# JeremyCCHsu/vae-npvc

Measured on AMD Instinct MI355X. Metric: SP frames/sec (train step: fwd+bwd+Adam), higher is better.
Workload: dtype f32 tensors and accumulation / bf16x2 operands (16 mantissa bits) on the matrix cores

## Files before the change

vae-npvc_amd/csrc/gfx950_layers.hip:

```cpp
#include <cstdlib>
#include <cstring>
#include <type_traits>

#include "gfx950_convgemm.h"
#include "gfx950_convwgrad.h"
#include "gfx950_dense.h"
#include "gfx950_elem.h"
#include "gfx950_tngemm.h"
#include "gfx950_toeplitz.h"
#include "gfx950_toep_bf16.h"
#include "gfx950_planegemm.h"
#include "gfx950_ntring.h"
#include "gfx950_viewconv.h"
#include "gfx950_fconv.h"
#include "gfx950_fwgrad.h"
#include "gfx950_fconv_r.h"
#include "gfx950_fbwd.h"
#include "gfx950_lnb_planes.h"
#include "kernels.h"

namespace vaenpvc {
namespace tuned {

#ifndef E1F_T
// ... 1016 lines not shown
    }
  } else generic::bwd_dec_layer(m, P, F, w, G, s, 2);

  const bool gd0_planes = !lnq && F >= 1024 && bwd_on(VAENPVC_SEL_DEC0) && bwd_on(VAENPVC_SEL_DEC1) && cw_bwd(CW_D0, F);
  const bool gd0_only_planes = gd0_planes && fcr_bwd(CV_D0G, F) && rt().planes <= 2;
  auto lnb_dec0 = [&](const float* dy0) {
    const ConvL& pl = m.dec[0];
    if (gd0_only_planes)
      for_planes([&](auto npl) {
        constexpr int NPL = decltype(npl)::value;
        VAENPVC_TIMED("lnb_dec0", s, (launch_ln_bwd_planes<LnbCfg<32, 57>, NPL, CL_GD0, false>(dy0, w.dec_a[0], w.dec_st[0], P + pl.gamma_off, P + pl.beta_off,
                                         w.d_dec_a[0], us(w.cl[CL_GD0]), cl_plane(CL_GD0, F), G + pl.gamma_off, G + pl.beta_off, G + pl.b_off,
                                         w.scratch + Pk::lnpart, F, LWGS, s)));
      });
    else if (gd0_planes)
      for_planes([&](auto npl) {
        constexpr int NPL = decltype(npl)::value;
        VAENPVC_TIMED("lnb_dec0", s, (launch_ln_bwd_planes<LnbCfg<32, 57>, NPL, CL_GD0, true>(dy0, w.dec_a[0], w.dec_st[0], P + pl.gamma_off, P + pl.beta_off,
                                         w.d_dec_a[0], us(w.cl[CL_GD0]), cl_plane(CL_GD0, F), G + pl.gamma_off, G + pl.beta_off, G + pl.b_off,
                                         w.scratch + Pk::lnpart, F, LWGS, s)));
      });
    else
      VAENPVC_TIMED("lnb_dec0", s, launch_ln_bwd<LnbCfg<32, 57>>(dy0, w.dec_a[0], w.dec_st[0], P + pl.gamma_off, P + pl.beta_off, w.d_dec_a[0],
                                       G + pl.gamma_off, G + pl.beta_off, G + pl.b_off, w.scratch + Pk::lnpart, F, LWGS, s, lnq));
  };
  if (bwd_on(VAENPVC_SEL_DEC1) && bwd_on(VAENPVC_SEL_DEC2) && fb_bwd(FB_D1, F)) {
    const ConvL& pl = m.dec[0];
    float* dy0 = dy_cur == w.dy_tmp ? w.d_dec_a[1] : w.dy_tmp;
    if (gd0_only_planes && !abf) {
      const int nwg = (int)fbwd_grid_d1(rt().planes, F);
      fused_bwd(FB_D1, 1, dy_cur, dy0, "dec1_bwd", us(w.cl[CL_GD0]), cl_plane(CL_GD0, F), w.scratch + Pk::lnpart);
      VAENPVC_TIMED("lnb_dec0", s, hipLaunchKernelGGL(k_ln_bwd_reduce, dim3(3 * 32), dim3(256), 0, s, w.scratch + Pk::lnpart, nwg, 32,
                                                       G + pl.gamma_off, G + pl.beta_off, G + pl.b_off));
    } else {
      fused_bwd(FB_D1, 1, dy_cur, dy0, "dec1_bwd");
      lnb_dec0(dy0);
    }
    dec_bias_done[0] = true;
  } else if (bwd_on(VAENPVC_SEL_DEC1)) {
    const ConvL &l = m.dec[1], &pl = m.dec[0];
    WgArgs a{w.d_dec_a[1], nullptr, nullptr, nullptr, w.dec_a[0], w.dec_st[0], P + pl.gamma_off, P + pl.beta_off,
             G + l.w_off, F, 0};
    const bool fg = fc_bwd(CV_D1G, F), vg = !fg && cv_bwd(CV_D1G, F), fw = fw_bwd(CW_D1, F), vw = !fw && cw_bwd(CW_D1, F);
    if (vg || vw) gsplit(CL_GD1, w.d_dec_a[1], "dec1_gsplit");
    if (vw && !fwd_planes(VAENPVC_SEL_DEC1, CV_D1F, F)) asplit(CL_YD0, w.dec_a[0], w.dec_st[0], &pl, "dec1_asplit");
    ready();
    if (fw) fwg(CW_D1, w.dec_a[0], w.dec_st[0], &pl, w.d_dec_a[1], nullptr, nullptr, G + l.w_off, "dec1_wgrad");
    else if (vw) vwgrad(CW_D1, G + l.w_off, "dec1_wgrad");
    else VAENPVC_TIMED("dec1_wgrad", s2, launch_convwgrad<WD1>(a, WGS, s2));
    if (!dec_bias_done[1]) generic::bias_grad(w.d_dec_a[1], G + l.b_off, F, l.cout, l.hout, s);
    if (fg) fdgrad(CV_D1G, w.d_dec_a[1], w.dy_tmp, "dec1_dgrad");
    else if (vg) vdgrad(CV_D1G, w.dy_tmp, "dec1_dgrad");
    else
    VAENPVC_TIMED("dec1_dgrad", s, launch_convgemm<GD1>(conv_args(w.d_dec_a[1], nullptr, nullptr, nullptr, P + l.w_off, nullptr,
                                                                  w.dy_tmp, F), nsplit_for<GD1>(F), s));
    lnb_dec0(w.dy_tmp);
    dec_bias_done[0] = true;
  } else generic::bwd_dec_layer(m, P, F, w, G, s, 1);

  const bool dh_planes = rt().d0g_planes && gd0_only_planes && fcr_otl(CV_D0G, rt().planes) && pg_step(VAENPVC_SEL_MERGE, F) && F >= 64;
  if (bwd_on(VAENPVC_SEL_DEC0)) {
    const ConvL& l = m.dec[0];
    WgArgs a{w.d_dec_a[0], nullptr, nullptr, nullptr, w.h, nullptr, nullptr, nullptr, G + l.w_off, F, 0};
    const bool rg = fcr_bwd(CV_D0G, F), vg = !rg && cv_bwd(CV_D0G, F), vw = cw_bwd(CW_D0, F);
    if ((vg || vw) && !gd0_planes) gsplit(CL_GD0, w.d_dec_a[0], "dec0_gsplit");
    if (vw && !fwd_planes(VAENPVC_SEL_DEC0, CV_D0F, F) && !d0f_leaves_planes(F)) asplit(CL_H, w.h, nullptr, nullptr, "dec0_asplit");
    ready();
    if (vw) vwgrad(CW_D0, G + l.w_off, "dec0_wgrad");
    else VAENPVC_TIMED("dec0_wgrad", s2, launch_convwgrad<WD0>(a, WGS, s2));
    if (!dec_bias_done[0]) generic::bias_grad(w.d_dec_a[0], G + l.b_off, F, l.cout, l.hout, s);
    if (rg) rdgrad(CV_D0G, w.scratch + Pk::cvw + cv_woff(CV_D0G), w.d_dec_a[0], w.d_h, "dec0_dgrad", gd0_only_planes ? w.cl[CL_GD0] : nullptr,
                   dh_planes ? w.pl_dh : nullptr, 1600);
    else if (vg) vdgrad(CV_D0G, w.d_h, "dec0_dgrad");
    else
    VAENPVC_TIMED("dec0_dgrad", s, (F < SMALL_BATCH_FRAMES ? launch_convgemm<GD0s>(conv_args(w.d_dec_a[0], nullptr, nullptr, nullptr, w.scratch + Pk::gd0,
                                                                  nullptr, w.d_h, F), nsplit_for<GD0s>(F), s) : launch_convgemm<GD0>(conv_args(w.d_dec_a[0], nullptr, nullptr, nullptr, w.scratch + Pk::gd0,
                                                                  nullptr, w.d_h, F), nsplit_for<GD0>(F), s)));
  } else generic::bwd_dec_layer(m, P, F, w, G, s, 0);
  if (lnq) flush_ln_reduce(*lnq, s);
  bucket(m.dec[0].w_off, m.n_params);

  if (bwd_on(VAENPVC_SEL_MERGE)) {
    const bool pgm = pg_step(VAENPVC_SEL_MERGE, F);
    if (pgm) {
      for_planes([&](auto npl) {
        constexpr int NPL = decltype(npl)::value;
        if (F >= 64) {
        int nch = 0;
        if (dh_planes) VAENPVC_TIMED("merge_dsplit", s, (nch = launch_segsum_planes<NPL, MERGE_NY>(us(w.pl_dh), (int64_t)F * 1600, y, 1539, 1600, F, w.dy_tmp, s)));
        else
        VAENPVC_TIMED("merge_dsplit", s, (nch = launch_split_segsum<NPL, MERGE_NY>(w.d_h, y, 1539, 1600, F, us(w.pl_dh), w.dy_tmp, s)));
        VAENPVC_TIMED("merge_segsum", s, launch_sum_parts(w.dy_tmp, nch, MERGE_NY * 1539, w.scratch + Pk::merge_s, s));
        } else {
        SplitArgs sa = split_args(w.d_h, 1539, 1600, F, us(w.pl_dh));
        VAENPVC_TIMED("merge_dsplit", s, launch_split<NPL>(sa, s));
        }
        ready();
        TnpArgs t = tnp_args(w.pl_z, 128, w.pl_dh, 1600, 128, 1539, F, G + m.wz_off, 1539);
        t.tn4 = bwd_on(VAENPVC_SEL_TN_W4);
        VAENPVC_TIMED("merge_wgrad", s2, (launch_gemm_tn<NPL, TN_EPI_PLAIN>(t, TN_WGS_DENSE, s2)));
      });
    } else {
    TnArgs a = tn_args(w.z, 128, w.d_h, 1539, 128, 1539, F, G + m.wz_off, 1539);
    ready();
    VAENPVC_TIMED("merge_wgrad", s2, launch_tngemm(a, false, kchunks_for(F, 13), s2));
    }
    float* Sg = w.scratch + Pk::merge_s;
    if (!(pgm && F >= 64)) {
      (void)hipMemsetAsync(Sg, 0, (size_t)MERGE_NY * 1539 * 4, s);
      int ch = cmax(1, cmin_(cdiv(F, 64), 128)), fc = cdiv(F, ch);
      VAENPVC_TIMED("merge_segsum", s, hipLaunchKernelGGL(k_segsum_atomic<MERGE_NY>, dim3((unsigned)cdiv(1539, 256), (unsigned)cdiv(F, fc)), dim3(256), 0, s,
                                                          w.d_h, y, 1539, F, fc, Sg));
    }
    const int nb_w = cdiv(128 * 1539, 256), nb_e = cdiv(MERGE_NY * 128, 4), nb_b = cdiv(1539, 256);
    VAENPVC_TIMED("merge_small", s, hipLaunchKernelGGL(k_merge_small<MERGE_NY>, dim3((unsigned)(nb_w + nb_e + nb_b)), dim3(256), 0, s, Sg, P + m.emb_off, P + m.wy_off, 128,
                       1539, G + m.wy_off, G + m.emb_off, G + m.bz_off, G + m.by_off, G + m.bm_off, nb_w, nb_e));
    if (pgm) {
      for_planes([&](auto npl) {
        constexpr int NPL = decltype(npl)::value;
        NtArgs a = nt_args(w.pl_dh, F, 1600, w.scratch + Pk::pg_mergeb, 128, 128, w.d_z, 128);
        VAENPVC_TIMED("merge_dgrad", s, launch_gemm_nt<NPL>(a, s));
      });
    } else {
      DenseArgs d = dense_args(w.d_h, w.scratch + Pk::merge_b, w.d_z, 128, F);
      if (F < SMALL_BATCH_FRAMES) {
        (void)hipMemsetAsync(w.d_z, 0, (size_t)F * 128 * 4, s);
        VAENPVC_TIMED("merge_dgrad", s, launch_densegemm<MergeBs>(d, s, 7));
      } else
      VAENPVC_TIMED("merge_dgrad", s, launch_densegemm<MergeB>(d, s));
    }
  } else generic::bwd_merge(m, P, y, F, w, G, s);
  bucket(m.wz_off, m.dec[0].w_off);

  const bool heads_tuned = bwd_on(VAENPVC_SEL_HEADS);
  const bool dz_planes = F >= 1024 && pg_step(VAENPVC_SEL_HEADS, F);
  if (heads_tuned) {
    const int rch = cmax(1, cmin_(cdiv(F, 32), 1024)), rfc = cdiv(F, rch);
    if (dz_planes)
      for_planes([&](auto npl) {
        VAENPVC_TIMED("reparam_bwd", s, hipLaunchKernelGGL((k_reparam_bwd_planes<decltype(npl)::value>), dim3((unsigned)cdiv(F, rfc)), dim3(256), 0, s, w.d_z, w.z_mu,
                           w.z_lv, eps, us(w.pl_dz), w.scratch + Pk::lnpart, (int)F, rfc, 1.0f / (float)F);
                      hipLaunchKernelGGL(k_colsum_part2, dim3(256), dim3(256), 0, s, w.scratch + Pk::lnpart, cdiv(F, rfc), G + m.bmu_off, G + m.blv_off));
      });
    else
    VAENPVC_TIMED("reparam_bwd", s, hipLaunchKernelGGL(k_reparam_bwd_colsum, dim3((unsigned)cdiv(F, rfc)), dim3(256), 0, s, w.d_z, w.z_mu, w.z_lv, eps, w.d_z_mu,
                       w.d_z_lv, G + m.bmu_off, G + m.blv_off, (int)F, rfc, 1.0f / (float)F));
  } else generic::bwd_reparam(m, eps, F, w, s);

  const bool da4_planes = !lnq && F >= 1024 && pg_step(VAENPVC_SEL_HEADS, F) && bwd_on(VAENPVC_SEL_ENC4) && fwd_on(VAENPVC_SEL_ENC4);
  const bool ge3_planes = !lnq && F >= 1024 && bwd_on(VAENPVC_SEL_ENC3) && bwd_on(VAENPVC_SEL_ENC4) && cv_bwd(CV_E3G, F) && cw_bwd(CW_E3, F);
  if (pg_step(VAENPVC_SEL_HEADS, F)) {
    const ConvL& l4 = m.enc[4];
    for_planes([&](auto npl) {
      constexpr int NPL = decltype(npl)::value;
      SplitArgs sa = split_args(w.d_z_mu, 256, 256, F, us(w.pl_dz));
      sa.k1 = 128;
      sa.ld1 = 128;
      sa.src2 = w.d_z_lv;
      sa.ld2 = 128;
      if (!dz_planes) VAENPVC_TIMED("heads_dsplit", s, launch_split<NPL>(sa, s));
      ready();
      TnpArgs t = tnp_args(w.pl_y4, 768, w.pl_dz, 256, 768, 256, F, G + m.wmu_off, 128);
      t.C2 = G + m.wlv_off;
      t.split = 128;
      t.tn4 = bwd_on(VAENPVC_SEL_TN_W4);
      VAENPVC_TIMED("heads_wgrad", s2, (launch_gemm_tn<NPL, TN_EPI_PLAIN>(t, TN_WGS_DENSE, s2)));
      NtArgs a = nt_args(w.pl_dz, F, 256, w.scratch + Pk::pg_headsb, 768, 768, w.dy_tmp, 768);
      VAENPVC_TIMED("heads_dgrad", s, launch_gemm_nt<NPL>(a, s));
    });
    if (da4_planes)
      for_planes([&](auto npl) {
        constexpr int NPL = decltype(npl)::value;
        VAENPVC_TIMED("lnb_enc4", s, (launch_ln_bwd_planes<LnbCfg<256, 3>, NPL, -1, false>(w.dy_tmp, w.enc_a[4], w.enc_st[4], P + l4.gamma_off, P + l4.beta_off,
                                         w.d_enc_a[4], us(w.pl_da4), (int64_t)F * 768, G + l4.gamma_off, G + l4.beta_off, G + l4.b_off,
                                         w.scratch + Pk::lnpart, F, LWGS, s)));
      });
    else
    VAENPVC_TIMED("lnb_enc4", s, launch_ln_bwd<LnbCfg<256, 3>>(w.dy_tmp, w.enc_a[4], w.enc_st[4], P + l4.gamma_off, P + l4.beta_off, w.d_enc_a[4],
                                     G + l4.gamma_off, G + l4.beta_off, G + l4.b_off, w.scratch + Pk::lnpart, F, LWGS, s, lnq));
    enc_bias_done[4] = true;
  } else if (bwd_on(VAENPVC_SEL_HEADS)) {
    const ConvL& l4 = m.enc[4];
    TnArgs a = tn_args(w.enc_a[4], 768, w.d_z_mu, 128, 768, 128, F, G + m.wmu_off, 128);
    a.st = w.enc_st[4];
    a.gamma = P + l4.gamma_off;
    a.beta = P + l4.beta_off;
    a.lndiv = 3;
    ready();
    VAENPVC_TIMED("heads_wgrad", s2, launch_tngemm(a, false, kchunks_for(F, 6), s2));
    a.Y = w.d_z_lv;
    a.C = G + m.wlv_off;
    launch_tngemm(a, false, kchunks_for(F, 6), s2);
    DenseArgs d = dense_args(w.d_z_mu, w.scratch + Pk::heads_b, w.dy_tmp, 768, F);
    d.in2 = w.d_z_lv;
    if (F < SMALL_BATCH_FRAMES) {
      (void)hipMemsetAsync(w.dy_tmp, 0, (size_t)F * 768 * 4, s);
      VAENPVC_TIMED("heads_dgrad", s, launch_densegemm<HeadsBs>(d, s, 4));
    } else
// ... 265 lines not shown
```

vae-npvc_amd/csrc/gfx950_planegemm.h:

```cpp
#pragma once
#include "gfx950_common.h"
#include "gfx950_toep_bf16.h"
#include "philox.h"

namespace vaenpvc {
namespace tuned {

constexpr int PG_KA = 64;

struct RowView {
  int R, fs, x0, step;
};
__device__ __forceinline__ int64_t view_off(const RowView& v, int r) {
  const int f = r / v.R, q = r - f * v.R;
  return (int64_t)f * v.fs + v.x0 + q * v.step;
}
static inline RowView plain_rows(int ld) { return RowView{0x7fffffff, 0, 0, ld}; }

struct SplitArgs {
  const float* src;
  const float* src2;
  int k1, ld1, ld2;
  const float* st;
  const float* gamma;
// ... 846 lines not shown
#pragma unroll
      for (int i = 0; i < 2; ++i)
#pragma unroll
        for (int j = 0; j < 2; ++j) acc[i][j] = mfma_bf16(fa[set][i][PR::A[t]], fb[set][j][PR::B[t]], acc[i][j]);
  };
  constexpr int NKS = NTA_KP / 16;
  auto tile_body = [&](int t, auto full_) __attribute__((always_inline)) {
    constexpr bool FULL = decltype(full_)::value;
    const int n0 = t * NT_BN;
#pragma unroll
    for (int p = 0; p < NPL; ++p)
#pragma unroll
      for (int q = 0; q < NQ; ++q) *reinterpret_cast<u32x4*>(sB + p * BPL + srow * NTA_RS + shalf * NTA_KP + q * 16) = rbq[p][q];
    if constexpr (rb) {
#pragma unroll
      for (int u = 0; u < NTB; ++u) Ts[tid + 256 * u] = tb[u];
    }
    const f32x4 bv = bv4;
    __syncthreads();
    gload(min(t + 1, ntn - 1));
    __builtin_amdgcn_sched_barrier(0);
#pragma unroll
    for (int i = 0; i < 2; ++i)
#pragma unroll
      for (int j = 0; j < 2; ++j) acc[i][j] = zero16();
    loadF(0, 0);
#pragma unroll
    for (int ks = 0; ks < NKS; ++ks) {
      if (ks + 1 < NKS) loadF((ks + 1) & 1, ks + 1);
      __builtin_amdgcn_sched_barrier(0);
      mm(ks & 1);
      __builtin_amdgcn_sched_barrier(0);
    }
    __syncthreads();
    float* ot = reinterpret_cast<float*>(sB);
#pragma unroll
    for (int j = 0; j < 2; ++j)
#pragma unroll
      for (int i = 0; i < 2; ++i)
#pragma unroll
        for (int reg = 0; reg < 16; ++reg)
          ot[(wm * 64 + i * 32 + acc_row(reg, lane)) * NT_EP_PITCH + wn * 64 + j * 32 + l31] = acc[i][j][reg];
    __syncthreads();
    const int pc = tid & 31, r0 = tid >> 5, n = n0 + pc * 4;
    float* cb = a.C + (int64_t)m0 * a.ldc + n;
#pragma unroll
    for (int i = 0; i < NT_BM / 8; ++i) {
      const int row = r0 + 8 * i;
      f32x4 v = *reinterpret_cast<const f32x4*>(ot + row * NT_EP_PITCH + pc * 4);
      v += bv;
      if constexpr (rb) v += *reinterpret_cast<const f32x4*>(Ts + ys[row] * 128 + pc * 4);
      float* o = cb + (int64_t)row * a.ldc;
      if (FULL || n + 3 < a.N) {
        *reinterpret_cast<f32x4_a4*>(o) = f32x4_a4{v[0], v[1], v[2], v[3]};
      } else {
#pragma unroll
        for (int k = 0; k < 4; ++k)
          if (n + k < a.N) o[k] = v[k];
      }
    }
    __syncthreads();
  };
  const int nfull = a.N / NT_BN;
  gload(0);
  tile_body(0, std::true_type{});
  for (int t = 1; t < nfull; ++t) tile_body(t, std::true_type{});
  if (nfull < ntn) tile_body(nfull, std::false_type{});
}
inline bool gemm_nt_ar_serves(const NtArgs& a) {
  return a.Kp == NTA_KP && a.M % NT_BM == 0 && !a.C2 && (!a.rowbias || (a.nrb <= NT_MAXRB && a.idx)) && a.N >= NT_BN;
}
template <int NPL>
inline void launch_gemm_nt_ar(const NtArgs& a, hipStream_t s) {
  if (a.rowbias) {
    rt().ensure_lds(reinterpret_cast<const void*>(&k_gemm_nt_ar<NPL, true>), nta_lds(NPL));
    hipLaunchKernelGGL((k_gemm_nt_ar<NPL, true>), dim3((unsigned)(a.M / NT_BM)), dim3(256), nta_lds(NPL), s, a);
  } else {
    rt().ensure_lds(reinterpret_cast<const void*>(&k_gemm_nt_ar<NPL, false>), nta_lds(NPL));
    hipLaunchKernelGGL((k_gemm_nt_ar<NPL, false>), dim3((unsigned)(a.M / NT_BM)), dim3(256), nta_lds(NPL), s, a);
  }
}


enum { TN_EPI_PLAIN = 0, TN_EPI_ENC4 = 1, TN_EPI_TRANS = 2 };
struct TnpArgs {
  const unsigned short* A;
  const unsigned short* B;
  int64_t a_plane, b_plane;
  RowView av, bv;
  int lda, ldb;
  int xcd;
  int tn4;
  int M, N, F, fchunk;
  float* C;
  float* C2;
  int split, ldc;
};
constexpr int TP_KF = 16;
template <int NPL, int TI, int TJ>
struct TnTile {
  static constexpr int BM = 64 * TI, BN = 128 * TJ;
  static constexpr int tn32_pitch(int w) { return ((w * 2 + 64) / 4) % 32 == 16 ? w * 2 + 64 : w * 2; }
  static constexpr int RSA = tn32_pitch(BM), RSB = tn32_pitch(BN);
  static_assert((RSA / 4) % 32 == 16 && (RSB / 4) % 32 == 16 && RSA % 16 == 0 && RSB % 16 == 0, "conflict-free row pitches");
  static constexpr int APL = TP_KF * RSA, BPL = TP_KF * RSB;
  static constexpr int BUF = NPL * (APL + BPL), LDS = 2 * BUF;
  static constexpr int APC = BM / 8, BPC = BN / 8;
};

template <int NPL, int EPI, int TI = 2, int TJ = 2>
__global__ void __launch_bounds__(512, NPL <= 2 ? 4 : 2) k_gemm_tn(TnpArgs a) {
  using T = TnTile<NPL, TI, TJ>;
  extern __shared__ __attribute__((aligned(16))) unsigned char smem[];
  constexpr int BUF = T::BUF;
  const int tid = threadIdx.x, lane = tid & 63, wave = tid >> 6, lh = lane >> 5, l31 = lane & 31;
  const int wr = wave >> 2, wc = wave & 3;
  const int ntm = cdiv(a.M, T::BM), ntt = ntm * cdiv(a.N, T::BN);
  const int wg = a.xcd ? xcd_contiguous(blockIdx.x, gridDim.x) : blockIdx.x;
  const int zc = wg / ntt, tl = wg - zc * ntt;
  const int m0 = (tl % ntm) * T::BM, n0 = (tl / ntm) * T::BN;
  const int fb = zc * a.fchunk, fe = min(a.F, fb + a.fchunk);
  const bool a_thr = tid < TP_KF * T::APC, b_thr = tid < TP_KF * T::BPC;
  const int arow = (tid / T::APC) & 15, apc = tid % T::APC;
  const int brow = (tid / T::BPC) & 15, bpc = tid % T::BPC;
  const int acol = cmin_(m0 * 2 + apc * 16, a.lda * 2 - 16);
  const int bcol = cmin_(n0 * 2 + bpc * 16, a.ldb * 2 - 16);
  const unsigned char* A8 = reinterpret_cast<const unsigned char*>(a.A);
  const unsigned char* B8 = reinterpret_cast<const unsigned char*>(a.B);
  u32x4 sta[NPL], stb[NPL];
  struct RowIt {
    unsigned off;
    int q;
  };
  auto row_init = [&](const RowView& v, int r, int colbytes) {
    RowIt it;
    const int f = r / v.R;
    it.q = r - f * v.R;
    it.off = (unsigned)(f * v.fs + v.x0 + it.q * v.step) * 2u + (unsigned)colbytes;
    return it;
  };
  const int adf = TP_KF / a.av.R, adq = TP_KF - adf * a.av.R, bdf = TP_KF / a.bv.R, bdq = TP_KF - bdf * a.bv.R;
  auto row_next = [&](const RowView& v, int df, int dq, RowIt& it) __attribute__((always_inline)) {
    int q = it.q + dq;
    const int carry = q >= v.R ? 1 : 0;
    q -= carry ? v.R : 0;
    it.off += (unsigned)(((df + carry) * v.fs + (q - it.q) * v.step) * 2);
    it.q = q;
  };
  RowIt ia = row_init(a.av, min(fb + arow, a.F - 1), acol), ib = row_init(a.bv, min(fb + brow, a.F - 1), bcol);
  auto gload = [&](int f0) __attribute__((always_inline)) {
    if (a_thr) {
#pragma unroll
      for (int p = 0; p < NPL; ++p) sta[p] = *reinterpret_cast<const u32x4*>(A8 + (size_t)p * a.a_plane * 2 + ia.off);
      if (f0 + TP_KF + arow < a.F) row_next(a.av, adf, adq, ia);
    }
    if (b_thr) {
#pragma unroll
      for (int p = 0; p < NPL; ++p) stb[p] = *reinterpret_cast<const u32x4*>(B8 + (size_t)p * a.b_plane * 2 + ib.off);
      if (f0 + TP_KF + brow < a.F) row_next(a.bv, bdf, bdq, ib);
    }
  };
  auto lstore = [&](int f0, int buf) __attribute__((always_inline)) {
    unsigned char* sA = smem + buf * BUF;
    unsigned char* sB = sA + NPL * T::APL;
    const u32x4 z = {0u, 0u, 0u, 0u};
    const bool tail = f0 + TP_KF > fe;
    if (a_thr) {
#pragma unroll
      for (int p = 0; p < NPL; ++p)
        *reinterpret_cast<u32x4*>(sA + p * T::APL + arow * T::RSA + apc * 16) = (tail && f0 + arow >= fe) ? z : sta[p];
    }
    if (b_thr) {
#pragma unroll
      for (int p = 0; p < NPL; ++p) *reinterpret_cast<u32x4*>(sB + p * T::BPL + brow * T::RSB + bpc * 16) = stb[p];
    }
  };
  const int trow = ((lane & 15) >> 2) + 8 * lh, tcol = 4 * (lane & 3) + 16 * ((lane >> 4) & 1);
  const int aoff = trow * T::RSA + (32 * TI * wr + tcol) * 2;
  const int boff = NPL * T::APL + trow * T::RSB + (32 * TJ * wc + tcol) * 2;
// ... 64 lines not shown
    for (int j = 0; j < TJ; ++j) {
      const int n = n0 + 32 * TJ * wc + 32 * j + l31;
      if (n >= a.N) continue;
#pragma unroll
      for (int reg = 0; reg < 16; ++reg) {
        const int m = m0 + 32 * TI * wr + 32 * i + acc_row(reg, lane);
        if (m >= a.M) continue;
        const float v = acc[i][j][reg];
        if constexpr (EPI == TN_EPI_ENC4) {
          const int c = m / 7, h = m - 7 * c, o = n / 3, j3 = n - 3 * o, t = h - 3 * j3 + 3;
          if (t >= 0 && t < 7) atomicAdd(a.C + ((t * 128 + c) * 256 + o), v);
        } else {
          if (a.C2 && n >= a.split) atomicAdd(a.C2 + (int64_t)m * a.ldc + (n - a.split), v);
          else atomicAdd(a.C + (int64_t)m * a.ldc + n, v);
        }
      }
    }
}

template <int NPL, int EPI, int TI, int TJ, int WR, int WC>
inline void launch_gemm_tn32(TnpArgs a, int target_wgs, hipStream_t s);
template <int NPL, int EPI, int TI = 2, int TJ = 2>
inline void launch_gemm_tn(TnpArgs a, int target_wgs, hipStream_t s) {
  if constexpr (NPL <= 2 && EPI != TN_EPI_TRANS && TI == 2 && TJ == 2) {
    if (a.tn4 && a.F >= 4096 && a.av.R >= a.F && a.bv.R >= a.F && cdiv(a.M, 256) * cdiv(a.N, 256) >= 8)
      return launch_gemm_tn4<NPL, EPI>(a, s);
  }
  if constexpr (NPL == 1) {
    return launch_gemm_tn32<NPL, EPI, TI, TJ, 2, 4>(a, target_wgs, s);
  } else {
    if constexpr (NPL == 2) {
      const bool many_tiles = cdiv(a.M, 64 * TI) * cdiv(a.N, 128 * TJ) > 8;
      if (!many_tiles) return launch_gemm_tn32<NPL, EPI, TI, TJ, 2, 4>(a, target_wgs, s);
    }
    using T = TnTile<NPL, TI, TJ>;
    rt().ensure_lds(reinterpret_cast<const void*>(&k_gemm_tn<NPL, EPI, TI, TJ>), T::LDS);
    const int tiles = cdiv(a.M, T::BM) * cdiv(a.N, T::BN);
    const int zc = cmax(1, cmin_(cdiv(a.F, 64), cdiv(target_wgs, tiles)));
    a.fchunk = rup(cdiv(a.F, zc), TP_KF);
    dim3 grid((unsigned)(cdiv(a.M, T::BM) * cdiv(a.N, T::BN) * cdiv(a.F, a.fchunk)));
    hipLaunchKernelGGL((k_gemm_tn<NPL, EPI, TI, TJ>), grid, dim3(512), T::LDS, s, a);
  }
}

constexpr int TP32_KF = 32;
template <int NPL, int TI, int TJ, int WR = 2, int WC = 4>
struct Tn32Tile {
  static constexpr int BM = 32 * TI * WR, BN = 32 * TJ * WC, NTHR = 64 * WR * WC;
  static constexpr int tn32_pitch(int w) { return ((w * 2 + 64) / 4) % 32 == 16 ? w * 2 + 64 : w * 2; }
  static constexpr int RSA = tn32_pitch(BM), RSB = tn32_pitch(BN);
  static_assert((RSA / 4) % 32 == 16 && (RSB / 4) % 32 == 16 && RSA % 16 == 0 && RSB % 16 == 0, "conflict-free row pitches");
  static constexpr int APL = TP32_KF * RSA, BPL = TP32_KF * RSB;
  static constexpr int BUF = NPL * (APL + BPL), LDS = 2 * BUF;
  static constexpr int APC = BM / 8, BPC = BN / 8;
};
#define TN32_INTERLEAVE(N, MASK, CNT)                        \
  _Pragma("unroll") for (int _i = 0; _i < (N); ++_i) {       \
    __builtin_amdgcn_sched_group_barrier(0x008, 1, 0);        \
    __builtin_amdgcn_sched_group_barrier((MASK), (CNT), 0);   \
  }

template <int NPL, int EPI, int TI = 2, int TJ = 2, int WR = 2, int WC = 4>
__global__ void __launch_bounds__((Tn32Tile<NPL, TI, TJ, WR, WC>::NTHR), (WR * WC <= 8 ? 2 : 1)) k_gemm_tn32(TnpArgs a) {
  static_assert(NPL <= 2, "three planes do not fit two 32-row buffers");
  using T = Tn32Tile<NPL, TI, TJ, WR, WC>;
  static_assert(TP32_KF * T::APC <= T::NTHR && 16 * T::BPC <= T::NTHR, "one staging piece of A, two of B per thread");
  extern __shared__ __attribute__((aligned(16))) unsigned char smem[];
  constexpr int BUF = T::BUF;
  const int tid = threadIdx.x, lane = tid & 63, wave = tid >> 6, lh = lane >> 5, l31 = lane & 31;
  const int wr = wave / WC, wc = wave % WC;
  const int ntm = cdiv(a.M, T::BM), ntt = ntm * cdiv(a.N, T::BN);
  const int wg = a.xcd ? xcd_contiguous(blockIdx.x, gridDim.x) : blockIdx.x;
  const int zc = wg / ntt, tl = wg - zc * ntt;
  const int m0 = (tl % ntm) * T::BM, n0 = (tl / ntm) * T::BN;
  const int fb = zc * a.fchunk, fe = min(a.F, fb + a.fchunk);
  const bool a_thr = tid < TP32_KF * T::APC, b_thr = tid < 16 * T::BPC;
  const int arow = (tid / T::APC) & 31, apc = tid % T::APC;
  const int brow = (tid / T::BPC) & 15, bpc = tid % T::BPC;
  const int acol = cmin_(m0 * 2 + apc * 16, a.lda * 2 - 16);
  const int bcol = cmin_(n0 * 2 + bpc * 16, a.ldb * 2 - 16);
  const unsigned char* A8 = reinterpret_cast<const unsigned char*>(a.A);
  const unsigned char* B8 = reinterpret_cast<const unsigned char*>(a.B);
  u32x4 sta[NPL], stb[NPL][2];
  struct RowIt {
    unsigned off;
    int q;
  };
  auto row_init = [&](const RowView& v, int r, int colbytes) {
    RowIt it;
    const int f = r / v.R;
    it.q = r - f * v.R;
    it.off = (unsigned)(f * v.fs + v.x0 + it.q * v.step) * 2u + (unsigned)colbytes;
    return it;
  };
  const int adf = TP32_KF / a.av.R, adq = TP32_KF - adf * a.av.R, bdf = TP32_KF / a.bv.R, bdq = TP32_KF - bdf * a.bv.R;
  auto row_next = [&](const RowView& v, int df, int dq, RowIt& it) __attribute__((always_inline)) {
    int q = it.q + dq;
    const int carry = q >= v.R ? 1 : 0;
    q -= carry ? v.R : 0;
    it.off += (unsigned)(((df + carry) * v.fs + (q - it.q) * v.step) * 2);
    it.q = q;
  };
  RowIt ia = row_init(a.av, min(fb + arow, a.F - 1), acol);
  RowIt ib0 = row_init(a.bv, min(fb + brow, a.F - 1), bcol), ib1 = row_init(a.bv, min(fb + brow + 16, a.F - 1), bcol);
  auto gload = [&](int f0) __attribute__((always_inline)) {
    if (a_thr) {
#pragma unroll
      for (int p = 0; p < NPL; ++p) sta[p] = *reinterpret_cast<const u32x4*>(A8 + (size_t)p * a.a_plane * 2 + ia.off);
      if (f0 + TP32_KF + arow < a.F) row_next(a.av, adf, adq, ia);
    }
    if (b_thr) {
#pragma unroll
      for (int p = 0; p < NPL; ++p) {
        stb[p][0] = *reinterpret_cast<const u32x4*>(B8 + (size_t)p * a.b_plane * 2 + ib0.off);
        stb[p][1] = *reinterpret_cast<const u32x4*>(B8 + (size_t)p * a.b_plane * 2 + ib1.off);
      }
      if (f0 + TP32_KF + brow < a.F) row_next(a.bv, bdf, bdq, ib0);
      if (f0 + TP32_KF + brow + 16 < a.F) row_next(a.bv, bdf, bdq, ib1);
    }
  };
  auto lstore = [&](int f0, int buf) __attribute__((always_inline)) {
    unsigned char* sA = smem + buf * BUF;
    unsigned char* sB = sA + NPL * T::APL;
    const u32x4 z = {0u, 0u, 0u, 0u};
    if (a_thr) {
      const bool zero = f0 + arow >= fe;
#pragma unroll
      for (int p = 0; p < NPL; ++p) *reinterpret_cast<u32x4*>(sA + p * T::APL + arow * T::RSA + apc * 16) = zero ? z : sta[p];
    }
    if (b_thr) {
#pragma unroll
      for (int p = 0; p < NPL; ++p) {
        *reinterpret_cast<u32x4*>(sB + p * T::BPL + brow * T::RSB + bpc * 16) = stb[p][0];
        *reinterpret_cast<u32x4*>(sB + p * T::BPL + (brow + 16) * T::RSB + bpc * 16) = stb[p][1];
      }
    }
  };
  const int trow = ((lane & 15) >> 2) + 8 * lh, tcol = 4 * (lane & 3) + 16 * ((lane >> 4) & 1);
  const int aoff = trow * T::RSA + (32 * TI * wr + tcol) * 2;
  const int boff = NPL * T::APL + trow * T::RSB + (32 * TJ * wc + tcol) * 2;
  f32x16 acc[TI][TJ];
#pragma unroll
  for (int i = 0; i < TI; ++i)
#pragma unroll
    for (int j = 0; j < TJ; ++j) acc[i][j] = zero16();
  u32x4 fa[2][TI][NPL], fbq[2][TJ][NPL];
  auto readF = [&](int set, int buf, int ks) __attribute__((always_inline)) {
    const unsigned char* sb = smem + buf * BUF;
#pragma unroll
    for (int i = 0; i < TI; ++i)
#pragma unroll
      for (int p = 0; p < NPL; ++p) fa[set][i][p] = tr_read8(sb + p * T::APL + ks * 16 * T::RSA + aoff + i * 64, 4 * T::RSA);
#pragma unroll
    for (int j = 0; j < TJ; ++j)
#pragma unroll
      for (int p = 0; p < NPL; ++p) fbq[set][j][p] = tr_read8(sb + p * T::BPL + ks * 16 * T::RSB + boff + j * 64, 4 * T::RSB);
  };
  constexpr int NTILE = TI * TJ, NHALF = NTILE >= 2 ? NTILE / 2 : 1;
  auto mma = [&](int set, int half) __attribute__((always_inline)) {
    using PR = Prod<NPL>;
#pragma unroll
    for (int t = 0; t < PR::N; ++t)
#pragma unroll
      for (int i = 0; i < TI; ++i)
#pragma unroll
        for (int j = 0; j < TJ; ++j) {
          const int id = i * TJ + j;
          if (NTILE >= 2 ? ((id & 1) != half) : (half != 0)) continue;
          if constexpr (EPI == TN_EPI_TRANS) acc[i][j] = mfma_bf16(fbq[set][j][PR::B[t]], fa[set][i][PR::A[t]], acc[i][j]);
          else acc[i][j] = mfma_bf16(fa[set][i][PR::A[t]], fbq[set][j][PR::B[t]], acc[i][j]);
        }
  };
  constexpr int NPROD = Prod<NPL>::N, NRD = (TI + TJ) * NPL * 2;
  if (fb < fe) {
    gload(fb);
    lstore(fb, 0);
    if (fb + TP32_KF < fe) gload(fb + TP32_KF);
  }
  __syncthreads();
  if (fb < fe) readF(0, 0, 0);
  int n = 0, f0 = fb;
  for (; f0 + TP32_KF < fe; f0 += TP32_KF, ++n) {
    const int buf = n & 1;
    readF(1, buf, 1);
    mma(0, 0);
    mma(0, 1);
    TN32_INTERLEAVE(NTILE * NPROD, 0x100, cdiv(NRD, NTILE * NPROD));
    __builtin_amdgcn_sched_barrier(0);
    lstore(f0 + TP32_KF, buf ^ 1);
    mma(1, 0);
    TN32_INTERLEAVE(NHALF * NPROD, 0x200, 1);
    __builtin_amdgcn_sched_barrier(0);
    if (f0 + 2 * TP32_KF < fe) gload(f0 + 2 * TP32_KF);
    __syncthreads();
    readF(0, buf ^ 1, 0);
    mma(1, 1);
    TN32_INTERLEAVE(NHALF * NPROD, 0x100, cdiv(NRD, NHALF * NPROD));
    __builtin_amdgcn_sched_barrier(0);
  }
  if (f0 < fe) {
    readF(1, n & 1, 1);
    mma(0, 0);
    mma(0, 1);
    mma(1, 0);
    mma(1, 1);
  }
  if constexpr (EPI == TN_EPI_TRANS) {
#pragma unroll
    for (int i = 0; i < TI; ++i)
#pragma unroll
      for (int j = 0; j < TJ; ++j) {
        const int m = m0 + 32 * TI * wr + 32 * i + l31;
        if (m >= a.M) continue;
#pragma unroll
        for (int reg = 0; reg < 16; ++reg) {
          const int nn = n0 + 32 * TJ * wc + 32 * j + acc_row(reg, lane);
          if (nn < a.N) atomicAdd(a.C + (int64_t)nn * a.ldc + m, acc[i][j][reg]);
        }
      }
    return;
  }
#pragma unroll
  for (int i = 0; i < TI; ++i)
#pragma unroll
    for (int j = 0; j < TJ; ++j) {
      const int nn = n0 + 32 * TJ * wc + 32 * j + l31;
      if (nn >= a.N) continue;
#pragma unroll
      for (int reg = 0; reg < 16; ++reg) {
        const int m = m0 + 32 * TI * wr + 32 * i + acc_row(reg, lane);
        if (m >= a.M) continue;
        const float v = acc[i][j][reg];
        if constexpr (EPI == TN_EPI_ENC4) {
          const int c = m / 7, h = m - 7 * c, o = nn / 3, j3 = nn - 3 * o, t = h - 3 * j3 + 3;
          if (t >= 0 && t < 7) atomicAdd(a.C + ((t * 128 + c) * 256 + o), v);
        } else {
          if (a.C2 && nn >= a.split) atomicAdd(a.C2 + (int64_t)m * a.ldc + (nn - a.split), v);
          else atomicAdd(a.C + (int64_t)m * a.ldc + nn, v);
        }
      }
    }
}

template <int NPL, int EPI, int TI, int TJ, int WR = 2, int WC = 4>
inline void launch_gemm_tn32(TnpArgs a, int target_wgs, hipStream_t s) {
  using T = Tn32Tile<NPL, TI, TJ, WR, WC>;
  rt().ensure_lds(reinterpret_cast<const void*>(&k_gemm_tn32<NPL, EPI, TI, TJ, WR, WC>), T::LDS);
  const int tiles = cdiv(a.M, T::BM) * cdiv(a.N, T::BN);
  const int zc = cmax(1, cmin_(cdiv(a.F, 128), cdiv(cmax(target_wgs / 2, 1), tiles)));
  a.fchunk = rup(cdiv(a.F, zc), TP32_KF);
  dim3 grid((unsigned)(tiles * cdiv(a.F, a.fchunk)));
  hipLaunchKernelGGL((k_gemm_tn32<NPL, EPI, TI, TJ, WR, WC>), grid, dim3(T::NTHR), T::LDS, s, a);
}

#ifndef VAENPVC_TN4_XCD
#define VAENPVC_TN4_XCD 1
#endif
constexpr int tn4_stage(int npl) { return npl * 2 * W4_APL; }
constexpr int tn4_lds(int npl) { return W4_NS * tn4_stage(npl) > 131072 ? W4_NS * tn4_stage(npl) : 131072; }
template <int NPL, int EPI>
__global__ void __launch_bounds__(256) k_gemm_tn4(TnpArgs a) {
  static_assert(NPL <= 2 && EPI != TN_EPI_TRANS, "two planes; plain and folded epilogues");
  extern __shared__ __attribute__((aligned(16))) unsigned char smem[];
  using PR = Prod<NPL>;
  constexpr int STAGE = tn4_stage(NPL), BOFF = NPL * W4_APL;
  constexpr int NB = 2 * NPL, NDMA = 2 * NB, NT8 = 8 * NPL, NM = 16 * PR::N;
  const int tid = threadIdx.x, lane = tid & 63, l31 = lane & 31, lh = lane >> 5;
  const int wave = __builtin_amdgcn_readfirstlane(tid >> 6);
  const int wr = wave >> 1, wc = wave & 1;
  const int ntm = cdiv(a.M, 256), ntt = ntm * cdiv(a.N, 256), nzc = gridDim.x / ntt;
  const int wgx = VAENPVC_TN4_XCD ? xcd_contiguous(blockIdx.x, gridDim.x) : -1;
  const int zc = VAENPVC_TN4_XCD ? wgx / ntt : blockIdx.x % nzc, tl = VAENPVC_TN4_XCD ? wgx - zc * ntt : blockIdx.x / nzc;
  const int m0 = (tl % ntm) * 256, n0 = (tl / ntm) * 256;
  const int fb = zc * a.fchunk, fe = min(a.F, fb + a.fchunk);
  if (fb >= fe) return;
  const int nst = (fe - fb + W4_KF - 1) / W4_KF;

  const unsigned char* A8 = reinterpret_cast<const unsigned char*>(a.A);
  const unsigned char* B8 = reinterpret_cast<const unsigned char*>(a.B);
  const unsigned lds0 = (unsigned)(unsigned long)(__attribute__((address_space(3))) unsigned char*)smem;
  const size_t arow = (size_t)a.lda * 2, brow = (size_t)a.ldb * 2;
  const unsigned char* src[NDMA];
  unsigned dst[NDMA];
#pragma unroll
  for (int k = 0; k < NB; ++k) {
    const int bid = wave * NB + k, pl = bid >> 3, fp = bid & 7, fr = 2 * fp + lh;
    const int gpc = l31 ^ ((fr & 3) << 2);
    src[2 * k] = A8 + (size_t)pl * a.a_plane * 2 + (size_t)(fb + fr) * arow + cmin_(m0 * 2 + gpc * 16, a.lda * 2 - 16);
    src[2 * k + 1] = B8 + (size_t)pl * a.b_plane * 2 + (size_t)(fb + fr) * brow + cmin_(n0 * 2 + gpc * 16, a.ldb * 2 - 16);
    dst[2 * k] = pl * W4_APL + fp * 1024;
    dst[2 * k + 1] = BOFF + pl * W4_APL + fp * 1024;
  }
  auto dma = [&](int g, int s, int slot) __attribute__((always_inline)) {
    const size_t off = (size_t)s * (W4_KF * ((g & 1) ? brow : arow));
    lds_dma16(src[g] + off, lds0 + slot * STAGE + dst[g]);
  };
  auto clear_tail = [&](int slot, int nv) __attribute__((always_inline)) {
    unsigned char* sb = smem + slot * STAGE;
    const u32x4 z = {0u, 0u, 0u, 0u};
    for (int i = tid; i < 2 * NPL * W4_KF * 32; i += 256)
      if (((i >> 5) & (W4_KF - 1)) >= nv) *reinterpret_cast<u32x4*>(sb + i * 16) = z;
    asm volatile("s_waitcnt lgkmcnt(0)" ::: "memory");
    __builtin_amdgcn_s_barrier();
  };
  const int last_nv = (fe - fb) - (nst - 1) * W4_KF;

  const int trow = ((lane & 15) >> 2) + 8 * lh, tcol = 4 * (lane & 3) + 16 * ((lane >> 4) & 1), s3 = trow & 3;
  int a_off[4], b_off[4];
#pragma unroll
  for (int r = 0; r < 4; ++r) {
    a_off[r] = trow * W4_RS + (16 * wr + ((r ^ s3) << 2) + (tcol >> 3)) * 16 + (tcol & 7) * 2;
    b_off[r] = BOFF + trow * W4_RS + (16 * wc + ((r ^ s3) << 2) + (tcol >> 3)) * 16 + (tcol & 7) * 2;
  }
  f32x16 acc[4][4];
#pragma unroll
  for (int ri = 0; ri < 4; ++ri)
#pragma unroll
    for (int cj = 0; cj < 4; ++cj) acc[ri][cj] = zero16();
  u32x4 fa[2][4][NPL], fq[2][4][NPL];
  auto rd = [&](int set, int slot, int j) __attribute__((always_inline)) {
    const unsigned char* sb = smem + slot * STAGE;
    if (j < 4 * NPL)
      fa[set][j / NPL][j % NPL] = tr_read8(sb + (j % NPL) * W4_APL + a_off[j / NPL], 4 * W4_RS);
    else if (j < NT8)
      fq[set][(j - 4 * NPL) / NPL][j % NPL] = tr_read8(sb + (j % NPL) * W4_APL + b_off[(j - 4 * NPL) / NPL], 4 * W4_RS);
  };
  auto mm = [&](int set, int m) __attribute__((always_inline)) {
    const int t = m >> 4, ri = (m >> 2) & 3, cj = m & 3;
    acc[ri][cj] = mfma_bf16(fa[set][ri][PR::A[t]], fq[set][cj][PR::B[t]], acc[ri][cj]);
  };
#pragma unroll
  for (int s = 0; s < 4; ++s)
#pragma unroll
    for (int g = 0; g < NDMA; ++g) dma(g, s, s);
  wait_vmcnt<2 * NDMA>();
  __builtin_amdgcn_s_barrier();
// ... 717 lines not shown
```

vae-npvc_amd/csrc/runtime.h:

```cpp
#pragma once
#include <hip/hip_runtime.h>

#include <cstdint>
#include <cstring>
#include <string>
#include <unordered_set>
#include <utility>
#include <vector>

namespace vaenpvc {

struct Runtime {
  unsigned fwd_mask = 0xffffffffu, bwd_mask = 0xffffffffu;
  int planes = 2;
  unsigned cv_sites() const { return planes == 1 ? 0xe2ceu : planes == 2 ? 0xc244u : 0x4u; }
  static constexpr unsigned FC_SITES = 0xdb1u;
  static constexpr unsigned FCR_SITES = 0x28au;
  static constexpr unsigned FW_SITES = 0x3fu;
  long fb_layers_env = -1;
  unsigned fb_layers() const { return fb_layers_env >= 0 ? (unsigned)fb_layers_env : 0x7u; }
  bool act_bf16 = false;
  int nt_ar = 0;
  int nt_ring = 1;
  int cg_sf_ring = 1;
  int cg_pf_ring = 0;
  bool dxh_skip = true;
  bool d0g_planes = true;
  int d2_lna = 1;
  bool d2_tail = false;
  bool toep_f32 = false;
  bool side_enabled = true;
  bool side_forced = false;
  int frame_max = 512;
  int64_t last_F = -1;
  int last_path = -1, last_planes = 0;
  unsigned last_fwd_mask = 0, last_bwd_mask = 0;
  const void* last_ws = nullptr;
  int64_t plz_F = -1;
  int64_t dxh_post_F = -1;
  int device = -1;
  hipStream_t s2 = nullptr;
  hipEvent_t ev[16] = {};
  int ev_next = 0;
  std::unordered_set<const void*> attr_done;
  void (*bucket_cb)(void* user, int32_t bucket, int64_t off, int64_t cnt, void* ready_stream) = nullptr;
  void* bucket_user = nullptr;
  int bucket_next = 0;
  std::string tag;
  std::vector<std::pair<hipEvent_t, hipEvent_t>> pool;
  size_t used = 0;

  void read_env();
  void bind_device();
  void release();
  void ensure_lds(const void* fn, int bytes);
  hipStream_t side_stream();
  void stream_dep(hipStream_t from, hipStream_t to);

  bool timer_match(const char* t) const {
    if (tag.empty()) return false;
    const size_t n = strlen(t);
    for (size_t p = tag.find(t); p != std::string::npos; p = tag.find(t, p + 1))
      if ((p == 0 || tag[p - 1] == ',') && (p + n == tag.size() || tag[p + n] == ',')) return true;
    return false;
  }
  void timer_begin(hipStream_t s);
  void timer_end(hipStream_t s);
};

Runtime& rt();
struct RtScope {
  Runtime* prev;
  explicit RtScope(Runtime* r);
  ~RtScope();
};

}
```

vae-npvc_amd/csrc/runtime.hip:

```cpp
#include "runtime.h"

#include <cstdlib>
#include <cstring>

namespace vaenpvc {

static thread_local Runtime* tl_rt = nullptr;
static Runtime g_detached;

Runtime& rt() { return tl_rt ? *tl_rt : g_detached; }
RtScope::RtScope(Runtime* r) : prev(tl_rt) { tl_rt = r; }
RtScope::~RtScope() { tl_rt = prev; }

void Runtime::read_env() {
  if (const char* e = getenv("VAENPVC_FWD_MASK")) fwd_mask = (unsigned)strtoul(e, nullptr, 0);
  if (const char* e = getenv("VAENPVC_BWD_MASK")) bwd_mask = (unsigned)strtoul(e, nullptr, 0);
  if (const char* e = getenv("VAENPVC_SIDE_STREAM")) {
    side_enabled = e[0] != '0';
    side_forced = side_enabled;
  }
  if (const char* e = getenv("VAENPVC_TOEP")) toep_f32 = !strcmp(e, "f32");
  if (const char* e = getenv("VAENPVC_D2_TAIL")) d2_tail = atoi(e) != 0;
  if (const char* e = getenv("VAENPVC_D2_LNA")) d2_lna = atoi(e);
  if (const char* e = getenv("VAENPVC_D0G_PLANES")) d0g_planes = atoi(e) != 0;
  if (const char* e = getenv("VAENPVC_DXH_SKIP")) dxh_skip = atoi(e) != 0;
  if (const char* e = getenv("VAENPVC_NT_RING")) nt_ring = atoi(e);
  if (const char* e = getenv("VAENPVC_CG_SF_RING")) cg_sf_ring = atoi(e);
  if (const char* e = getenv("VAENPVC_CG_PF_RING")) cg_pf_ring = atoi(e);
  if (const char* e = getenv("VAENPVC_NT_AR")) nt_ar = atoi(e);
  if (const char* e = getenv("VAENPVC_FRAME_MAX")) frame_max = atoi(e) < 0 ? 0 : (atoi(e) > 1024 ? 1024 : atoi(e));
  if (const char* e = getenv("VAENPVC_FB_LAYERS")) fb_layers_env = (long)strtoul(e, nullptr, 0);
  if (const char* e = getenv("VAENPVC_ACT_BF16")) act_bf16 = atoi(e) != 0;
  if (const char* e = getenv("VAENPVC_PLANES")) {
    int p = atoi(e);
    if (p >= 1 && p <= 3) planes = p;
  }
}

void Runtime::release() {
  if (s2) {
    (void)hipStreamSynchronize(s2);
    (void)hipStreamDestroy(s2);
    for (auto& e : ev)
      if (e) (void)hipEventDestroy(e);
  }
  s2 = nullptr;
  for (auto& e : ev) e = nullptr;
  ev_next = 0;
  for (auto& p : pool) {
    (void)hipEventDestroy(p.first);
    (void)hipEventDestroy(p.second);
  }
  pool.clear();
  used = 0;
  attr_done.clear();
}

void Runtime::bind_device() {
  int d = -1;
  if (hipGetDevice(&d) != hipSuccess) return;
  if (d == device) return;
  if (device >= 0) {
    int cur = d;
    (void)hipSetDevice(device);
    release();
    (void)hipSetDevice(cur);
  }
  device = d;
}

void Runtime::ensure_lds(const void* fn, int bytes) {
  if (attr_done.count(fn)) return;
  (void)hipFuncSetAttribute(fn, hipFuncAttributeMaxDynamicSharedMemorySize, bytes);
  attr_done.insert(fn);
}

hipStream_t Runtime::side_stream() {
  if (!side_enabled) return nullptr;
  if (s2) return s2;
  if (hipStreamCreateWithFlags(&s2, hipStreamNonBlocking) != hipSuccess) {
    s2 = nullptr;
    side_enabled = false;
    return nullptr;
  }
  for (auto& e : ev) (void)hipEventCreateWithFlags(&e, hipEventDisableTiming);
  return s2;
}

void Runtime::stream_dep(hipStream_t from, hipStream_t to) {
  hipEvent_t e = ev[ev_next];
  ev_next = (ev_next + 1) % 16;
  (void)hipEventRecord(e, from);
  (void)hipStreamWaitEvent(to, e, 0);
}

static const size_t kPoolMax = 16384;
void Runtime::timer_begin(hipStream_t s) {
  if (used >= kPoolMax) return;
  if (used >= pool.size()) {
    hipEvent_t a, b;
    (void)hipEventCreate(&a);
    (void)hipEventCreate(&b);
    pool.emplace_back(a, b);
  }
  (void)hipEventRecord(pool[used].first, s);
}
void Runtime::timer_end(hipStream_t s) {
// ... 7 lines not shown
```

Baseline: 5.799 million.

## Fuse merge one-hot segment sum into the merge weight-gradient TN GEMM

Adds a one-hot epilogue to the tn32 plane GEMM. Besides the weight gradient, each wave builds a bf16 one-hot operand from the speaker labels staged in LDS and runs an extra MFMA against the dh tiles, then atomically adds the per-speaker column sums into the segment-sum buffer. This replaces the separate split-segsum and sum-parts kernels on the main stream, and moves the small merge kernel to the side stream. The cost is an extra MFMA per k-step, atomics from the m0==0 tiles, a memset, and the one-hot sums now using bf16-rounded dh instead of f32.

```diff
diff --git a/vae-npvc_amd/csrc/gfx950_layers.hip b/vae-npvc_amd/csrc/gfx950_layers.hip
--- a/vae-npvc_amd/csrc/gfx950_layers.hip
+++ b/vae-npvc_amd/csrc/gfx950_layers.hip
@@ -1122,7 +1122,23 @@
 
   if (bwd_on(VAENPVC_SEL_MERGE)) {
     const bool pgm = pg_step(VAENPVC_SEL_MERGE, F);
-    if (pgm) {
+    float* Sg = w.scratch + Pk::merge_s;
+    const bool s_gemm = pgm && F >= 64 && rt().merge_s_gemm && rt().d0g_planes && gemm_tn_onehot_serves(rt().planes, 128, MERGE_NY);
+    if (s_gemm) {
+      for_planes([&](auto npl) {
+        constexpr int NPL = decltype(npl)::value;
+        if constexpr (NPL <= 2) {
+          if (!dh_planes) VAENPVC_TIMED("merge_dsplit", s, launch_split<NPL>(split_args(w.d_h, 1539, 1600, F, us(w.pl_dh)), s));
+          (void)hipMemsetAsync(Sg, 0, (size_t)MERGE_NY * 1539 * 4, s);
+          ready();
+          TnpArgs t = tnp_args(w.pl_z, 128, w.pl_dh, 1600, 128, 1539, F, G + m.wz_off, 1539);
+          t.oh_idx = y;
+          t.oh_n = MERGE_NY;
+          t.Coh = Sg;
+          VAENPVC_TIMED("merge_wgrad", s2, (launch_gemm_tn_onehot<NPL>(t, TN_WGS_DENSE, s2)));
+        }
+      });
+    } else if (pgm) {
       for_planes([&](auto npl) {
         constexpr int NPL = decltype(npl)::value;
         if (F >= 64) {
@@ -1145,7 +1161,6 @@
     ready();
     VAENPVC_TIMED("merge_wgrad", s2, launch_tngemm(a, false, kchunks_for(F, 13), s2));
     }
-    float* Sg = w.scratch + Pk::merge_s;
     if (!(pgm && F >= 64)) {
       (void)hipMemsetAsync(Sg, 0, (size_t)MERGE_NY * 1539 * 4, s);
       int ch = cmax(1, cmin_(cdiv(F, 64), 128)), fc = cdiv(F, ch);
@@ -1153,7 +1168,8 @@
                                                           w.d_h, y, 1539, F, fc, Sg));
     }
     const int nb_w = cdiv(128 * 1539, 256), nb_e = cdiv(MERGE_NY * 128, 4), nb_b = cdiv(1539, 256);
-    VAENPVC_TIMED("merge_small", s, hipLaunchKernelGGL(k_merge_small<MERGE_NY>, dim3((unsigned)(nb_w + nb_e + nb_b)), dim3(256), 0, s, Sg, P + m.emb_off, P + m.wy_off, 128,
+    hipStream_t sm = s_gemm ? s2 : s;
+    VAENPVC_TIMED("merge_small", sm, hipLaunchKernelGGL(k_merge_small<MERGE_NY>, dim3((unsigned)(nb_w + nb_e + nb_b)), dim3(256), 0, sm, Sg, P + m.emb_off, P + m.wy_off, 128,
                        1539, G + m.wy_off, G + m.emb_off, G + m.bz_off, G + m.by_off, G + m.bm_off, nb_w, nb_e));
     if (pgm) {
       for_planes([&](auto npl) {
diff --git a/vae-npvc_amd/csrc/gfx950_planegemm.h b/vae-npvc_amd/csrc/gfx950_planegemm.h
--- a/vae-npvc_amd/csrc/gfx950_planegemm.h
+++ b/vae-npvc_amd/csrc/gfx950_planegemm.h
@@ -952,7 +952,7 @@
 }
 
 
-enum { TN_EPI_PLAIN = 0, TN_EPI_ENC4 = 1, TN_EPI_TRANS = 2 };
+enum { TN_EPI_PLAIN = 0, TN_EPI_ENC4 = 1, TN_EPI_TRANS = 2, TN_EPI_ONEHOT = 3 };
 struct TnpArgs {
   const unsigned short* A;
   const unsigned short* B;
@@ -965,6 +965,9 @@
   float* C;
   float* C2;
   int split, ldc;
+  const int64_t* oh_idx;
+  int oh_n;
+  float* Coh;
 };
 constexpr int TP_KF = 16;
 template <int NPL, int TI, int TJ>
@@ -1195,6 +1198,13 @@
   const unsigned char* A8 = reinterpret_cast<const unsigned char*>(a.A);
   const unsigned char* B8 = reinterpret_cast<const unsigned char*>(a.B);
   u32x4 sta[NPL], stb[NPL][2];
+  constexpr bool OH = EPI == TN_EPI_ONEHOT;
+  static_assert(!OH || (TJ == 2 && WR == 2), "one-hot rows: the wave rows deal the column tiles");
+  typedef int i32x4 __attribute__((ext_vector_type(4)));
+  int* ysm = reinterpret_cast<int*>(smem + 2 * BUF);
+  int ohy = -1;
+  f32x16 acc_oh = zero16();
+  u32x4 foh[2];
   struct RowIt {
     unsigned off;
     int q;
@@ -1217,6 +1227,10 @@
   RowIt ia = row_init(a.av, min(fb + arow, a.F - 1), acol);
   RowIt ib0 = row_init(a.bv, min(fb + brow, a.F - 1), bcol), ib1 = row_init(a.bv, min(fb + brow + 16, a.F - 1), bcol);
   auto gload = [&](int f0) __attribute__((always_inline)) {
+    if (OH && tid < TP32_KF) {
+      const int64_t yy = a.oh_idx[min(f0 + tid, fe - 1)];
+      ohy = f0 + tid >= fe ? -1 : (int)(yy < 0 ? 0 : (yy >= a.oh_n ? a.oh_n - 1 : yy));
+    }
     if (a_thr) {
 #pragma unroll
       for (int p = 0; p < NPL; ++p) sta[p] = *reinterpret_cast<const u32x4*>(A8 + (size_t)p * a.a_plane * 2 + ia.off);
@@ -1241,6 +1255,7 @@
 #pragma unroll
       for (int p = 0; p < NPL; ++p) *reinterpret_cast<u32x4*>(sA + p * T::APL + arow * T::RSA + apc * 16) = zero ? z : sta[p];
     }
+    if (OH && tid < TP32_KF) ysm[buf * TP32_KF + tid] = ohy;
     if (b_thr) {
 #pragma unroll
       for (int p = 0; p < NPL; ++p) {
@@ -1268,6 +1283,14 @@
     for (int j = 0; j < TJ; ++j)
 #pragma unroll
       for (int p = 0; p < NPL; ++p) fbq[set][j][p] = tr_read8(sb + p * T::BPL + ks * 16 * T::RSB + boff + j * 64, 4 * T::RSB);
+    if constexpr (OH) {
+      const int* yp = ysm + buf * TP32_KF + ks * 16 + 8 * lh;
+      const i32x4 y0 = *reinterpret_cast<const i32x4*>(yp), y1 = *reinterpret_cast<const i32x4*>(yp + 4);
+      foh[set][0] = (y0[0] == l31 ? 0x3f80u : 0u) | (y0[1] == l31 ? 0x3f800000u : 0u);
+      foh[set][1] = (y0[2] == l31 ? 0x3f80u : 0u) | (y0[3] == l31 ? 0x3f800000u : 0u);
+      foh[set][2] = (y1[0] == l31 ? 0x3f80u : 0u) | (y1[1] == l31 ? 0x3f800000u : 0u);
+      foh[set][3] = (y1[2] == l31 ? 0x3f80u : 0u) | (y1[3] == l31 ? 0x3f800000u : 0u);
+    }
   };
   constexpr int NTILE = TI * TJ, NHALF = NTILE >= 2 ? NTILE / 2 : 1;
   auto mma = [&](int set, int half) __attribute__((always_inline)) {
@@ -1283,6 +1306,12 @@
           if constexpr (EPI == TN_EPI_TRANS) acc[i][j] = mfma_bf16(fbq[set][j][PR::B[t]], fa[set][i][PR::A[t]], acc[i][j]);
           else acc[i][j] = mfma_bf16(fa[set][i][PR::A[t]], fbq[set][j][PR::B[t]], acc[i][j]);
         }
+    if constexpr (OH) {
+      if (half == 1) {
+#pragma unroll
+        for (int p = 0; p < NPL; ++p) acc_oh = mfma_bf16(foh[set], wr ? fbq[set][1][p] : fbq[set][0][p], acc_oh);
+      }
+    }
   };
   constexpr int NPROD = Prod<NPL>::N, NRD = (TI + TJ) * NPL * 2;
   if (fb < fe) {
@@ -1353,18 +1382,34 @@
         }
       }
     }
+  if constexpr (OH) {
+    const int nn = n0 + 32 * TJ * wc + 32 * wr + l31;
+    if (m0 == 0 && nn < a.N) {
+#pragma unroll
+      for (int reg = 0; reg < 16; ++reg) {
+        const int k = acc_row(reg, lane);
+        if (k < a.oh_n) atomicAdd(a.Coh + (int64_t)k * a.ldc + nn, acc_oh[reg]);
+      }
+    }
+  }
 }
 
 template <int NPL, int EPI, int TI, int TJ, int WR = 2, int WC = 4>
 inline void launch_gemm_tn32(TnpArgs a, int target_wgs, hipStream_t s) {
   using T = Tn32Tile<NPL, TI, TJ, WR, WC>;
-  rt().ensure_lds(reinterpret_cast<const void*>(&k_gemm_tn32<NPL, EPI, TI, TJ, WR, WC>), T::LDS);
+  constexpr int LDS = T::LDS + (EPI == TN_EPI_ONEHOT ? 2 * TP32_KF * 4 : 0);
+  rt().ensure_lds(reinterpret_cast<const void*>(&k_gemm_tn32<NPL, EPI, TI, TJ, WR, WC>), LDS);
   const int tiles = cdiv(a.M, T::BM) * cdiv(a.N, T::BN);
   const int zc = cmax(1, cmin_(cdiv(a.F, 128), cdiv(cmax(target_wgs / 2, 1), tiles)));
   a.fchunk = rup(cdiv(a.F, zc), TP32_KF);
   dim3 grid((unsigned)(tiles * cdiv(a.F, a.fchunk)));
-  hipLaunchKernelGGL((k_gemm_tn32<NPL, EPI, TI, TJ, WR, WC>), grid, dim3(T::NTHR), T::LDS, s, a);
-}
+  hipLaunchKernelGGL((k_gemm_tn32<NPL, EPI, TI, TJ, WR, WC>), grid, dim3(T::NTHR), LDS, s, a);
+}
+template <int NPL>
+inline void launch_gemm_tn_onehot(const TnpArgs& a, int target_wgs, hipStream_t s) {
+  launch_gemm_tn32<NPL, TN_EPI_ONEHOT, 2, 2, 2, 4>(a, target_wgs, s);
+}
+inline bool gemm_tn_onehot_serves(int npl, int M, int oh_n) { return npl <= 2 && M <= 128 && oh_n >= 1 && oh_n <= 32; }
 
 #ifndef VAENPVC_TN4_XCD
 #define VAENPVC_TN4_XCD 1
diff --git a/vae-npvc_amd/csrc/runtime.h b/vae-npvc_amd/csrc/runtime.h
--- a/vae-npvc_amd/csrc/runtime.h
+++ b/vae-npvc_amd/csrc/runtime.h
@@ -26,6 +26,7 @@
   int cg_pf_ring = 0;
   bool dxh_skip = true;
   bool d0g_planes = true;
+  bool merge_s_gemm = true;
   int d2_lna = 1;
   bool d2_tail = false;
   bool toep_f32 = false;
diff --git a/vae-npvc_amd/csrc/runtime.hip b/vae-npvc_amd/csrc/runtime.hip
--- a/vae-npvc_amd/csrc/runtime.hip
+++ b/vae-npvc_amd/csrc/runtime.hip
@@ -23,6 +23,7 @@
   if (const char* e = getenv("VAENPVC_D2_TAIL")) d2_tail = atoi(e) != 0;
   if (const char* e = getenv("VAENPVC_D2_LNA")) d2_lna = atoi(e);
   if (const char* e = getenv("VAENPVC_D0G_PLANES")) d0g_planes = atoi(e) != 0;
+  if (const char* e = getenv("VAENPVC_MERGE_S_GEMM")) merge_s_gemm = atoi(e) != 0;
   if (const char* e = getenv("VAENPVC_DXH_SKIP")) dxh_skip = atoi(e) != 0;
   if (const char* e = getenv("VAENPVC_NT_RING")) nt_ring = atoi(e);
   if (const char* e = getenv("VAENPVC_CG_SF_RING")) cg_sf_ring = atoi(e);
```

Result: no change. 5.831 million (median of 6 runs) (+0.6%).
